# nelpy/ghost

Hardware: AMD Instinct MI355X
Metric: Msamples/s CWT (128ch x 1e6 samp x 100 scales); % HBM roofline; 1/2/4/8 GPU (higher is better)
Workload: dtype f32

## Files before the change

ghost_amd/csrc/api.cpp:

```cpp
#include <hip/hip_runtime.h>

#include <algorithm>
#include <cmath>
#include <cstdio>
#include <cstdlib>
#include <cstring>
#include <exception>
#include <map>
#include <new>
#include <string>
#include <vector>

#include "../../include/ghostcwt.h"
#include "../../include/ghostcwt_debug.h"
#include <memory>

#include "host_out.h"
#include "interp.h"
#include "kernels.h"
#include "morse_exact.h"
#include "options.h"
#include "planner.h"

using namespace gcwt;
// ... 18 lines not shown
  try {
    return body();
  } catch (const std::bad_alloc&) {
    return set_err(GCWT_ERR_NOMEM, "out of host memory");
  } catch (const std::exception& e) {
    return set_err(GCWT_ERR_INVALID, std::string("internal error: ") + e.what());
  } catch (...) {
    return set_err(GCWT_ERR_INVALID, "internal error");
  }
}

#define HIP_TRY(call)                                  \
  do {                                                 \
    hipError_t e_ = (call);                            \
    if (e_ != hipSuccess) return hip_err(e_, #call);   \
  } while (0)

struct EpochDev {
  SynthItemDev* items = nullptr;
  int n_items = 0;
  SynthLevelDev* levels = nullptr;
  Synth7Item* items7 = nullptr;
  Synth7Level* levels7 = nullptr;
  int n_items7 = 0;
  Synth7Item* items7w = nullptr;
  int n_items7w = 0;
  Synth7Item* items7n = nullptr;
  int n_items7n = 0;
  SynthiItem* items_i = nullptr;
  SynthiLevel* levels_i = nullptr;
  int n_items_i = 0;
  SynthpItem* items_p[2] = {nullptr, nullptr};
  SynthpLevel* levels_p = nullptr;
  int n_items_p[2] = {0, 0};
  PredLevel* pred_levels = nullptr;
};

constexpr int64_t kFullbandCacheBytes = (int64_t)16 << 30;

enum Stage { ST_MEAN = 0, ST_FWD, ST_DECIM, ST_BLOCK, ST_SYNTH, ST_DIRECT, ST_FULLBAND, ST_INTERP, ST_BLOCKCONV, ST_COUNT };

}

struct gcwt_plan {
  HostPlan hp;
  bool uploaded = false;
  int profiling = 0;
  int synth_cols = 32;
  int synth7_narrow_r = 2;
  bool fuse_blocks = true;
  int synth_kernel = 7;
  bool prune_inputs = true;
  bool fast_fft = true;
  int drop_stores = 0;
  bool clock_probe = false;
  bool use_synth16 = false;
  int device = -1;
  hipStream_t stream = nullptr;
  hipStream_t aux[2] = {nullptr, nullptr};
  bool level_streams = true;
  bool use_synthp = false;
  bool use_graphs = true;
  bool fullband4 = true;
  int fullband_group = 0;
  int64_t fullband_cache_cap = 0;
  bool hfull_cache_full = false;
  int synth7_order = 0;
  int synthp_help = -1;
  int synthp_lgnb = -1;
  int interp_lgnb = -1;
  int interp_grid = -1;
  bool last_fold = false;
  bool fold_mean = true;
  bool synth_streams = false;
  hipStream_t cur = nullptr;
  bool high_precision = true;
  double2* d_y = nullptr;
  int64_t y_stride = 0;
  double2* d_tw64 = nullptr;
  float2* d_x = nullptr;
  float2* d_xr = nullptr;
  float2* d_xb = nullptr;
  float2* d_bank = nullptr;
  float* d_gain = nullptr;
  float* d_gain_lv = nullptr;
  float2* d_half_tw = nullptr;
  float2* d_psi = nullptr;
  float2* d_psi_tail = nullptr;
  float2* d_psi_lit = nullptr;
  unsigned long long* d_probe = nullptr;
  double* d_amps = nullptr;
  float2* d_xs = nullptr;
  int64_t xs_stride = 0;
  float2* d_z = nullptr;
  int64_t z_half = 0;
  int z_sets = 1;
  float2* d_hfull = nullptr;
  std::map<std::pair<int, int>, float2*> hfull_cache;
  int64_t hfull_cache_bytes = 0;
  float2* d_tw4096 = nullptr;
  float2* d_tw256 = nullptr;
  float2* d_level_tw = nullptr;
  double* d_sums = nullptr;
  int32_t* d_scale_list = nullptr;
  int n_listed = 0;
  int32_t* d_scale_aux = nullptr;
// ... 196 lines not shown
  if (!free_bytes || !total_bytes) return set_err(GCWT_ERR_INVALID, "NULL argument");
  HIP_TRY(hipMemGetInfo(free_bytes, total_bytes));
  return GCWT_OK;
}
int gcwt_device_malloc(void** ptr, size_t bytes) { HIP_TRY(hipMalloc(ptr, bytes ? bytes : 1)); return GCWT_OK; }
int gcwt_device_free(void* ptr) { HIP_TRY(hipFree(ptr)); return GCWT_OK; }
int gcwt_memcpy_h2d(void* dst, const void* src, size_t bytes) {
  HIP_TRY(hipMemcpy(dst, src, bytes, hipMemcpyHostToDevice)); return GCWT_OK;
}
int gcwt_memcpy_d2h(void* dst, const void* src, size_t bytes) {
  HIP_TRY(hipMemcpy(dst, src, bytes, hipMemcpyDeviceToHost)); return GCWT_OK;
}
int gcwt_device_memset(void* dst, int value, size_t bytes) {
  HIP_TRY(hipMemset(dst, value, bytes)); return GCWT_OK;
}
int gcwt_device_synchronize(void) { HIP_TRY(hipDeviceSynchronize()); return GCWT_OK; }
int gcwt_host_alloc(void** ptr, size_t bytes) {
  if (!ptr) return set_err(GCWT_ERR_INVALID, "NULL argument");
  HIP_TRY(hipHostMalloc(ptr, bytes ? bytes : 1, hipHostMallocDefault));
  return GCWT_OK;
}
int gcwt_host_free(void* ptr) { HIP_TRY(hipHostFree(ptr)); return GCWT_OK; }
int gcwt_rows_to_host(const float* d_src, int64_t src_pitch, int64_t n_rows, int64_t row_elems, void* dst,
                      int64_t dst_pitch, int flags) {
  return guarded([&] {
    if (!d_src || !dst) return set_err(GCWT_ERR_INVALID, "NULL argument");
    if (n_rows < 0 || row_elems < 0 || src_pitch < row_elems || dst_pitch < row_elems)
      return set_err(GCWT_ERR_INVALID, "bad rectangle (rows, elements per row, pitches)");
    if (!(flags & GCWT_HOST_PINNED) && dst_pitch != row_elems)
      return set_err(GCWT_ERR_INVALID, "a destination that is not page-locked takes dense rows (dst_pitch = row_elems)");
    HIP_TRY(rows_to_host(d_src, src_pitch, n_rows, row_elems, dst, dst_pitch, (flags & GCWT_OUT_F64) != 0,
                         (flags & GCWT_HOST_PINNED) != 0));
    return (int)GCWT_OK;
  });
}

static int gcwt_plan_create_impl(gcwt_plan** out, const gcwt_params* params) {
  if (!out || !params) return set_err(GCWT_ERR_INVALID, "NULL argument");
  *out = nullptr;
  std::unique_ptr<gcwt_plan> owner(new (std::nothrow) gcwt_plan());
  gcwt_plan* p = owner.get();
  if (!p) return set_err(GCWT_ERR_NOMEM, "out of host memory");
  std::string err;
  int rc = build_host_plan(*params, &p->hp, &err);
  if (rc != GCWT_OK) return set_err(rc, err);
  p->hp.prm.freqs_hz = p->hp.freqs.data();
  p->hp.prm.epoch_bounds = p->hp.bounds.data();
  p->hp.prm.n_epochs = (int32_t)(p->hp.bounds.size() / 2);
  p->device = params->device;
  p->high_precision = p->hp.high_precision;
  p->use_synth16 = option_or("synth16", 0) == 1;
  p->synth_cols = option_or("synth_cols", 32) == 16 ? 16 : 32;
  p->synth7_narrow_r = (int)option_or("synth7_narrow_r", 2);
  p->fuse_blocks = option_or("fuse_blocks", 1) != 0;
  p->prune_inputs = option_or("prune_inputs", 1) != 0;
  p->fast_fft = option_or("slow_fft", 0) == 0;
  p->level_streams = option_or("level_streams", 1) != 0;
  if (option_is_set("interp_grid")) p->interp_grid = option_or("interp_grid", 0) != 0;
  p->synth_streams = option_or("synth_streams", 0) != 0;
  p->fold_mean = option_or("fold_mean", 1) != 0;
  p->interp_lgnb = (int)option_or("interp_lgnb", -1);
  p->use_synthp = kMeasureBuild && option_or("synthp", 0) != 0;
  p->synthp_lgnb = (int)option_or("synthp_lgnb", -1);
  p->synthp_help = (int)option_or("synthp_help", -1);
  p->use_graphs = option_or("graphs", 1) != 0;
  p->synth7_order = (int)option_or("synth7_order", 0);
  p->auto_threshold = 1e-9f * (float)option_or("auto_threshold_ppb", 1500);
  p->kappa_eps = 1e-9f * (float)option_or("auto_kappa_ppb", 160);
  p->oob_tol = 1e-12f * (float)option_or("auto_oob_ppt", 25000);
  p->fullband_group = (int)option_or("fullband_group", 0);
  p->fullband4 = option_or("fullband4", 1) != 0;
  p->synth_kernel = kMeasureBuild && option_or("synth_kernel", 7) == 8 ? 8 : 7;
  p->drop_stores = kMeasureBuild && option_is_set("synth_drop_stores") ? (int)std::max<long long>(1, option_or("synth_drop_stores", 1)) : 0;
  p->clock_probe = kMeasureBuild && option_is_set("clock_probe");
  for (const auto& s : p->hp.scales)
    if (s.method == GCWT_SCALE_DIRECT) p->max_direct_len = std::max(p->max_direct_len, s.length);
  *out = owner.release();
  return GCWT_OK;
}

void gcwt_plan_destroy(gcwt_plan* plan) {
  if (!plan) return;
  if (plan->uploaded || plan->stream) {
    if (plan->device >= 0) (void)hipSetDevice(plan->device);
    free_dev(plan);
  }
  delete plan;
}

int gcwt_plan_get_info(const gcwt_plan* plan, gcwt_plan_info* info) {
  if (!plan || !info) return set_err(GCWT_ERR_INVALID, "NULL argument");
  const HostPlan& hp = plan->hp;
  info->abi_version = GCWT_ABI_VERSION;
  info->n_levels = (int32_t)hp.levels.size();
  info->n_direct = hp.n_direct;
  info->n_spectral = (int32_t)hp.scales.size() - hp.n_direct - hp.n_fullband - hp.n_blockconv;
  info->n_fullband = hp.n_fullband;
  info->n_blockconv = hp.n_blockconv;
  info->reserved = 0;
  info->n_interp = 0;
  for (const auto& l : hp.levels)
    if (level_kernel(plan, l) == LK_INTERP) info->n_interp += (int32_t)l.scales.size();
  info->block = hp.block;
  int r = 1;
  for (const auto& l : hp.levels) r = std::max(r, l.decimation);
  info->max_decimation = r;
// ... 757 lines not shown
      ap.row_len = row_len;
      ap.xr = p->d_xr;
      ap.xr_cstride = hp.max_xr;
      ap.xb_scale = (float)(1.0 / ((double)hp.block * (double)Pt));
      ap.n_scales = S;
      ap.channels_fastest = p->interp_grid >= 0 ? p->interp_grid : (slots <= 32 ? 1 : 0);
      if (dev.n_items_p[k] > 65535) ap.channels_fastest = 0;
      ap.flags = 0;
      ap.seg = sout;
      p->cur = si;
#ifdef GCWT_MEASURE
      if (strided) return set_err(GCWT_ERR_UNSUPPORTED, "output stride with the pipelined interpolating kernel");
      RUN(ST_INTERP, launch_synthp(mode, ap, dev.n_items_p[k], slots, k == 1, si));
#else
      return set_err(GCWT_ERR_INVALID, "internal: a level planned for the measure build's pipelined kernel");
#endif
      p->cur = nullptr;
    }
    if (dev.n_items > 0) {
      SynthArgs a{};
      a.xb = p->d_xb;
      a.bank = p->d_bank;
      a.tw256 = p->d_tw256;
      a.level_tw = p->d_level_tw;
      a.items = dev.items;
      a.levels = dev.levels;
      a.out = dout;
      a.xb_cstride = hp.max_xb;
      a.row_len = row_len;
      a.n_scales = S;
      a.seg = sout;
      RUN(ST_SYNTH, launch_synth(mode, a, dev.n_items, slots, st));
    }
    for (int variant = 0; variant < 3; ++variant) {
      const int wide = variant == 2;
      const int cols7 = variant == 0 ? 16 : p->synth_cols;
      const int n7 = variant == 0 ? dev.n_items7n : wide ? dev.n_items7w : dev.n_items7;
      if (n7 == 0) continue;
      Synth7Args a7{};
      a7.xb = p->d_xb;
      a7.bank = p->d_bank;
      a7.tw256 = p->d_tw256;
      a7.level_tw = p->d_level_tw;
      a7.items = variant == 0 ? dev.items7n : wide ? dev.items7w : dev.items7;
      a7.levels = dev.levels7;
      a7.scale_list = p->d_scale_list;
      a7.gain = p->d_gain;
      a7.gain_lv = p->d_gain_lv;
      a7.level_half_tw = p->d_half_tw;
      a7.out = dout;
      a7.xb_cstride = hp.max_xb;
      a7.row_len = row_len;
      a7.n_scales = S;
      a7.drop_stores = p->drop_stores;
      a7.seg = sout;
      a7.clock_probe = p->d_probe;
      if (fused_blocks) {
        a7.xr = p->d_xr;
        a7.xr_cstride = hp.max_xr;
        a7.xb_scale = (float)(1.0 / ((double)hp.block * (double)Pt));
      }
      if (strided) {
        RUN(ST_SYNTH, launch_synth7s(mode, cols7, a7, n7, slots, st));
        continue;
      }
#ifdef GCWT_MEASURE
      if (p->synth_kernel == 8 && variant == 1)
        RUN(ST_SYNTH, launch_synth8(mode, p->synth_cols, a7, n7, slots, st));
      else
#endif
        RUN(ST_SYNTH, launch_synth7(mode, cols7, wide != 0, a7, n7, slots, st));
    }
    if (si != st) {
      hipEvent_t interp_done;
      int rc_ = get_event(p, &interp_done);
      if (rc_) return rc_;
      he = hipEventRecord(interp_done, si);
      if (he == hipSuccess) he = hipStreamWaitEvent(st, interp_done, 0);
      if (he != hipSuccess) return hip_err(he, "synthesis join");
    }
    if (p->detect && p->d_y) {
      hipEvent_t pred_done;
      int rc_ = get_event(p, &pred_done);
      if (rc_) return rc_;
      he = hipEventRecord(pred_done, p->det_stream);
      if (he == hipSuccess) he = hipStreamWaitEvent(st, pred_done, 0);
      if (he != hipSuccess) return hip_err(he, "detector join");
    }
    if (p->profiling && !hp.levels.empty()) p->last.synth_launches++;
    auto response = [&](int i, int scratch, const float2** h_out) -> int {
      const auto cached = p->hfull_cache.find({i, P1});
      if (cached != p->hfull_cache.end()) { *h_out = cached->second; return GCWT_OK; }
      float2* dst = p->d_hfull + (int64_t)scratch * hp.max_p;
      float2* keep = nullptr;
      const int64_t bytes = (int64_t)sizeof(float2) * P;
      if (!p->hfull_cache_full && p->hfull_cache_bytes + bytes <= p->fullband_cache_cap) {
        if (hipMalloc((void**)&keep, (size_t)bytes) == hipSuccess) dst = keep;
        else {
          (void)hipGetLastError();
          p->hfull_cache_full = true;
        }
      }
      {
        SpanGuard sg_(p, ST_FULLBAND);
        int rc_ = sg_.rc;
        if (!rc_) {
// ... 453 lines not shown

int gcwt_get_timings(const gcwt_plan* p, gcwt_timings* t) {
  if (!p || !t) return set_err(GCWT_ERR_INVALID, "NULL argument");
  if (!p->have_timings) return set_err(GCWT_ERR_INVALID, "no profiled execute yet");
  *t = p->last;
  return GCWT_OK;
}

int gcwt_plan_create(gcwt_plan** out, const gcwt_params* params) {
  return guarded([&] { return gcwt_plan_create_impl(out, params); });
}

int gcwt_plan_upload(gcwt_plan* p) {
  return guarded([&] { return gcwt_plan_upload_impl(p); });
}

int gcwt_execute(gcwt_plan* p, const void* x, void* out, int flags) {
  return guarded([&] { return gcwt_execute_impl(p, x, out, flags); });
}

int gcwt_execute_block(gcwt_plan* p, const void* x, void* out, int64_t start, int64_t length,
                       int flags) {
  return guarded([&] { return gcwt_execute_block_impl(p, x, out, start, length, flags); });
}


int gcwt_debug_measure_build(void) { return kMeasureBuild ? 1 : 0; }

int gcwt_debug_level_count(const gcwt_plan* p) { return p ? (int)p->hp.levels.size() : -1; }

int gcwt_debug_level_info(const gcwt_plan* p, int epoch, int level, int32_t* decimation,
                          int32_t* halo, int32_t* hop, int32_t* nblk, int64_t* m) {
  if (!p) return set_err(GCWT_ERR_INVALID, "NULL plan");
  if (epoch < 0 || epoch >= (int)p->hp.epochs.size() || level < 0 ||
      level >= (int)p->hp.levels.size())
    return set_err(GCWT_ERR_INVALID, "epoch/level out of range");
  const LevelPlan& lp = p->hp.levels[level];
  const EpochLevel& el = p->hp.epochs[epoch].lv[level];
  if (decimation) *decimation = lp.decimation;
  if (halo) *halo = lp.halo;
  if (hop) *hop = lp.hop;
  if (nblk) *nblk = el.nblk;
  if (m) *m = el.m;
  return GCWT_OK;
}

int gcwt_debug_level_band_shift(const gcwt_plan* p, int level, int32_t* shift) {
  if (!p || !shift) return set_err(GCWT_ERR_INVALID, "NULL argument");
  if (level < 0 || level >= (int)p->hp.levels.size()) return set_err(GCWT_ERR_INVALID, "level out of range");
  *shift = p->hp.levels[level].band_shift;
  return GCWT_OK;
}

int gcwt_debug_set_option(const char* name, int64_t value, int clear) {
  const int rc = option_set(name, (long long)value, clear != 0);
  if (rc == -1) return set_err(GCWT_ERR_INVALID, std::string("unknown option: ") + (name ? name : "(null)"));
  if (rc == -2) return set_err(GCWT_ERR_UNSUPPORTED, std::string("option ") + name + " exists in libghostcwt_measure.so only");
  return GCWT_OK;
}

int gcwt_debug_level_low_cut(const gcwt_plan* p, int level, double* theta_cut) {
  if (!p || !theta_cut) return set_err(GCWT_ERR_INVALID, "NULL argument");
  if (level < 0 || level >= (int)p->hp.levels.size()) return set_err(GCWT_ERR_INVALID, "level out of range");
  const LevelPlan& own = p->hp.levels[p->hp.levels[level].xr_owner];
  *theta_cut = p->hp.high_precision && own.band_shift == 0 ? own.taper_hi : 0.0;
  return GCWT_OK;
}

int gcwt_debug_scale_theta_lo(const gcwt_plan* p, double* theta_lo) {
  if (!p || !theta_lo) return set_err(GCWT_ERR_INVALID, "NULL argument");
  for (size_t i = 0; i < p->hp.scales.size(); ++i) theta_lo[i] = p->hp.scales[i].theta_lo;
  return GCWT_OK;
}

int gcwt_debug_mean_folded(const gcwt_plan* p) {
  if (!p) return set_err(GCWT_ERR_INVALID, "NULL plan");
  return p->last_fold ? 1 : 0;
}

int gcwt_debug_graph_state(const gcwt_plan* p) {
  if (!p) return set_err(GCWT_ERR_INVALID, "NULL plan");
  return p->graph_failed ? -1 : p->graph_exec ? 1 : 0;
}

int gcwt_debug_blockconv_groups(const gcwt_plan* p, int32_t* first, int32_t* count, int32_t* hop, int32_t* back,
                                int32_t* order, int max_groups, int max_order) {
  if (!p) return set_err(GCWT_ERR_INVALID, "NULL plan");
  const HostPlan& hp = p->hp;
  const int n = (int)hp.bc_groups.size();
  for (int g = 0; g < n && g < max_groups; ++g) {
    if (first) first[g] = hp.bc_groups[g].first;
    if (count) count[g] = hp.bc_groups[g].count;
    if (hop) hop[g] = hp.bc_groups[g].hop;
    if (back) back[g] = hp.bc_groups[g].back;
  }
  if (order) for (int k = 0; k < hp.n_blockconv && k < max_order; ++k) order[k] = hp.bc_order[k];
  return n;
}

int gcwt_debug_interp_level(const gcwt_plan* p, int level, int32_t* q, int32_t* factor, double* alpha,
                            double* err_bound, float* coef, int64_t max_floats) {
  if (!p) return set_err(GCWT_ERR_INVALID, "NULL plan");
  if (level < 0 || level >= (int)p->hp.levels.size()) return set_err(GCWT_ERR_INVALID, "level out of range");
  const LevelPlan& lp = p->hp.levels[level];
  const bool on = level_kernel(p, lp) == LK_INTERP;
  if (q) *q = on ? lp.interp_q : 0;
// ... 108 lines not shown
```

ghost_amd/csrc/kernels.h:

```cpp
#pragma once
#include <hip/hip_runtime.h>

#include <algorithm>
#include <cstdint>

#include "../../include/ghostcwt.h"

namespace gcwt {

constexpr int kRowLenDev = 4096;

#ifdef GCWT_MEASURE
constexpr bool kMeasureBuild = true;
#else
constexpr bool kMeasureBuild = false;
#endif

struct BankScale {
  double omega;
  double half_delay;
  int64_t length;
  int64_t amp_offset;
  int32_t bin_lo, n_bins;
  int32_t decimation;
// ... 59 lines not shown
  int32_t decimation, hop, halo, blk_base;
  int64_t xb_offset;
  int64_t tw_offset;
};

struct SynthArgs {
  const float2* xb;
  const float2* bank;
  const float2* tw256;
  const float2* level_tw;
  const SynthItemDev* items;
  const SynthLevelDev* levels;
  float* out;
  int64_t xb_cstride;
  int64_t row_len;
  int32_t n_scales;
  int32_t pad;
  SegOut seg;
};

struct Synth7Item {
  int32_t level, blk0, rtile, pad;
};

struct Synth7Level {
  int32_t decimation, log2r, hop, halo, nblk, n_scales, scale_offset, blk_base;
  int32_t n_plain;
  int32_t half_offset;
  int32_t band_shift;
  int32_t pad1;
  int64_t xb_offset;
  int64_t tw_offset;
  int64_t xr_offset;
  int64_t m_mask;
};

struct Synth7Args {
  const float2* xb;
  const float2* bank;
  const float2* tw256;
  const float2* level_tw;
  const Synth7Item* items;
  const Synth7Level* levels;
  const int32_t* scale_list;
  const float* gain;
  const float* gain_lv;
  const float2* level_half_tw;
  float* out;
  int64_t xb_cstride;
  int64_t row_len;
  const float2* xr;
  int64_t xr_cstride;
  float xb_scale;
  int32_t pad0;
  unsigned long long* clock_probe;
  int32_t n_scales;
  int32_t drop_stores;
  SegOut seg;
};

hipError_t launch_synth7(int mode, int ncol, bool wide_halo, const Synth7Args& a, int n_items, int n_channels,
                         hipStream_t st);
hipError_t launch_synth7s(int mode, int ncol, const Synth7Args& a, int n_items, int n_channels, hipStream_t st);

struct SynthiItem {
  int32_t level, blk0;
  int32_t pass0, n_pass;
  int32_t wt_lo, wt_hi;
};
struct SynthiLevel {
  int32_t decimation, q, log2q, factor;
  int32_t hop, halo, nblk, n_scales, scale_offset, blk_base;
  int32_t log2nb, taps;
  int64_t tw_offset;
  int64_t xr_offset;
  int64_t m_mask;
  int64_t coef_offset;
};
struct SynthiArgs {
  const float2* tw256;
  const float2* level_tw;
  const SynthiItem* items;
  const SynthiLevel* levels;
  const int32_t* scale_list;
  const int32_t* scale_aux;
  const float* gain;
  const float* coef;
  float* out;
  int64_t row_len;
  const float2* xr;
  int64_t xr_cstride;
  float xb_scale;
  int32_t n_scales;
  int32_t channels_fastest;
  SegOut seg;
};
hipError_t launch_synthi(int mode, const SynthiArgs& a, int n_items, int n_channels, hipStream_t st);
hipError_t launch_synthis(int mode, const SynthiArgs& a, int n_items, int n_channels, hipStream_t st);
constexpr int kSynthpThreads = 512;
constexpr int kSynthpProducers = 2;
constexpr int kSynthpSlots = 4;
constexpr int kSynthpMaxFactor = 256;
struct SynthpItem {
  int32_t level, blk0;
  int32_t round0, n_rounds;
};
struct SynthpLevel {
// ... 180 lines not shown
```

ghost_amd/csrc/options.cpp:

```cpp
#include "options.h"

#include <cctype>
#include <cstdlib>
#include <cstring>
#include <map>
#include <mutex>
#include <string>

#include "kernels.h"

namespace gcwt {
namespace {

const char* const kSelect[] = {"synth16", "synth_cols", "fuse_blocks", "slow_fft", "level_streams", "interp_grid",
                               "synth_streams", "interp_lgnb", "merge_levels", "split_levels", "interp",
                               "batch_bytes", "stage_floats", "fullband_group", "blockconv",
                               "direct_max_len", "graphs", "plan_threads", "fullband_cache_mb", "auto_threshold_ppb", "auto_kappa_ppb", "auto_oob_ppt", "synth7_order", "host_widen", "host_threads", "fullband4", "cu_count", "synth7_narrow_r", "fold_mean"};
const char* const kMeasureOnly[] = {"halo_margin", "interp_q", "interp_taps", "interp_min_r", "prune_inputs", "clock_phases",
                                    "synth_kernel", "synth_drop_stores", "clock_probe", "synthi_pad_kb",
                                    "synthp", "synthp_lgnb", "synthp_help"};
const char* const kEnvBudgets[] = {"batch_bytes", "stage_floats"};

std::mutex g_mu;
std::map<std::string, long long>& table() {
  static std::map<std::string, long long> t;
  return t;
}

template <size_t N>
bool in_list(const char* name, const char* const (&list)[N]) {
  for (const char* s : list)
    if (!strcmp(s, name)) return true;
  return false;
}

bool from_env(const char* name, long long* v) {
  std::string var = "GHOSTCWT_";
  for (const char* c = name; *c; ++c) var.push_back((char)toupper((unsigned char)*c));
  const char* e = getenv(var.c_str());
  if (!e) return false;
  *v = *e ? atoll(e) : 1;
  return true;
}

bool lookup(const char* name, long long* v) {
  {
    std::lock_guard<std::mutex> lock(g_mu);
    auto it = table().find(name);
    if (it != table().end()) { *v = it->second; return true; }
  }
  if (kMeasureBuild || in_list(name, kEnvBudgets)) return from_env(name, v);
  return false;
}

}

long long option_or(const char* name, long long dflt) {
  long long v;
  return lookup(name, &v) ? v : dflt;
}

bool option_is_set(const char* name) {
  long long v;
  return lookup(name, &v);
}

int option_set(const char* name, long long value, bool clear) {
  if (!name) return -1;
  const bool measure_only = in_list(name, kMeasureOnly);
  if (!measure_only && !in_list(name, kSelect)) return -1;
// ... 9 lines not shown
```

ghost_amd/csrc/planner.cpp:

```cpp
#include "planner.h"
#include "interp.h"
#include "morse_exact.h"
#include "options.h"

#include <algorithm>
#include <climits>
#include <cstdlib>
#include <cmath>
#include <map>
#include <atomic>
#include <mutex>
#include <new>
#include <thread>

namespace gcwt {

static int exact_method(const HostPlan& hp, int64_t length) {
  if (length <= hp.direct_max_len) return GCWT_SCALE_DIRECT;
  if (length <= hp.blockconv_max_len) return GCWT_SCALE_BLOCKCONV;
  return GCWT_SCALE_FULLBAND;
}
static bool uses_segment_fft(int method) { return method == GCWT_SCALE_SPECTRAL || method == GCWT_SCALE_FULLBAND; }

static void plan_blockconv(HostPlan* hp, bool rebalance) {
// ... 693 lines not shown
    if (sp.method != GCWT_SCALE_SPECTRAL) continue;
    const int r = sp.decimation;
    if (r > r_cap) return fail(GCWT_ERR_UNSUPPORTED, "internal: decimation beyond the shortest FFT");
    int halo = std::max((int)std::ceil(sp.support / (double)r) + halo_margin(), 16);
    if (r == 2) halo += halo & 1;
    const std::pair<int, int> key(r, sp.theta_neg > 0.0 && halo > 48 ? 2 : (split && halo > 16 ? 1 : 0));
    auto it = level_of.find(key);
    if (it == level_of.end()) {
      LevelPlan lp;
      lp.decimation = r;
      const int idx = (int)hp->levels.size();
      if (!owner_of_r.count(r)) owner_of_r[r] = idx;
      lp.xr_owner = owner_of_r[r];
      level_of[key] = idx;
      hp->levels.push_back(lp);
      it = level_of.find(key);
    }
    sp.level = it->second;
    LevelPlan& lp = hp->levels[sp.level];
    lp.scales.push_back(i);
    lp.halo = std::max(lp.halo, halo);
  }
  {
    std::map<int, int> shift_of_r;
    for (const LevelPlan& lp : hp->levels) {
      const double delta = 2.0 * M_PI / ((double)B * lp.decimation);
      int& shift = shift_of_r[lp.decimation];
      for (int i : lp.scales)
        if (hp->scales[i].theta_neg > 0.0)
          shift = std::max(shift, (int)std::ceil(hp->scales[i].theta_neg / delta));
    }
    for (LevelPlan& lp : hp->levels) {
      const double delta = 2.0 * M_PI / ((double)B * lp.decimation);
      const int g = std::max(1, lp.decimation / 16);
      const int shift = (shift_of_r[lp.decimation] + g - 1) / g * g;
      lp.band_shift = shift;
      for (int i : lp.scales)
        if (hp->scales[i].theta_hi > (double)(B - shift) * delta * (1.0 + 1e-12))
          return fail(GCWT_ERR_UNSUPPORTED, "internal: a scale's band does not fit its level's shifted band");
      if (shift > 0 && lp.scales.size() > 256)
        return fail(GCWT_ERR_UNSUPPORTED, "more than 256 heavy-tailed scales in one decimation level");
    }
  }
  if (hp->high_precision) {
    std::vector<double> lo(hp->levels.size(), 1e30);
    for (const LevelPlan& lp : hp->levels) {
      double& o = lo[(size_t)lp.xr_owner];
      if (lp.band_shift > 0) o = 0.0;
      for (int i : lp.scales) o = std::min(o, hp->scales[i].theta_lo);
    }
    for (size_t l = 0; l < hp->levels.size(); ++l)
      hp->levels[l].taper_hi = hp->levels[l].xr_owner == (int)l && lo[l] < 1e29 ? lo[l] : 0.0;
  }
  for (LevelPlan& lp : hp->levels) {
    lp.hop = B - 2 * lp.halo;
    if (lp.hop < 32)
      return fail(GCWT_ERR_UNSUPPORTED,
                  "internal: a spectral scale does not fit its 256-sample decimated block");
    lp.fast = lp.halo <= 48 && lp.scales.size() <= 256;
    if (!lp.fast) hp->halo_static = false;
    lp.twiddle_offset = hp->level_twiddle_total;
    hp->level_twiddle_total += (int64_t)kSynthCols * lp.decimation;
  }
  {
    if (option_or("interp", 1) != 0) {
      const size_t nl = hp->levels.size();
      std::vector<std::vector<float>> coef(nl);
      const unsigned n_thr = (unsigned)std::min<size_t>(nl, std::min<unsigned>((unsigned)std::max<long long>(1, option_or("plan_threads", 8)), std::max(1u, std::thread::hardware_concurrency())));
      if (n_thr <= 1) {
        for (size_t l = 0; l < nl; ++l) plan_interp_level(hp, &hp->levels[l], &coef[l]);
      } else {
        std::atomic<size_t> next{0};
        std::atomic<bool> failed{false};
        auto work = [&]() {
          try {
            for (size_t l = next++; l < nl; l = next++) plan_interp_level(hp, &hp->levels[l], &coef[l]);
          } catch (...) {
            failed = true;
          }
        };
        std::vector<std::thread> pool;
        try {
          for (unsigned k = 1; k < n_thr; ++k) pool.emplace_back(work);
        } catch (...) {
        }
        work();
        for (std::thread& t : pool) t.join();
        if (failed) throw std::bad_alloc();
      }
      for (size_t l = 0; l < nl; ++l) {
        if (hp->levels[l].interp_q <= 0 || coef[l].empty()) continue;
        hp->levels[l].coef_offset = (int64_t)hp->interp_coef.size();
        hp->interp_coef.insert(hp->interp_coef.end(), coef[l].begin(), coef[l].end());
      }
    }
  }

  for (const EpochPlan& ep : hp->epochs) {
    if (ep.long_a == 1) continue;
    if (!hp->high_precision)
      return fail(GCWT_ERR_UNSUPPORTED, "FFT lengths above 2^22 (kernels of millions of taps) need precision = high");
    if (hp->n_fullband > 0)
      return fail(GCWT_ERR_UNSUPPORTED, "FFT lengths above 2^22 cannot serve full-band scales (heavy-tailed wavelet at very low frequencies)");
    for (const LevelPlan& lp : hp->levels) {
      const int64_t m = ep.p / lp.decimation;
      if (lp.band_shift > 0 || lp.decimation < 2 * ep.long_a ||
          (lp.decimation / ep.long_a > kMaxTwoPassDecimation && m > 8192))
// ... 90 lines not shown
```

ghost_amd/csrc/planner.h:

```cpp
#pragma once
#include <cstdint>
#include <string>
#include <vector>

#include "../../include/ghostcwt.h"

namespace gcwt {

constexpr int kRowLen = 4096;
constexpr int kMaxP1 = 1024;
constexpr int kMaxFftLog2 = 24;
constexpr int kMaxDecimation = 16384;
constexpr int kMaxBatch = 16;
constexpr int kMaxTwoPassDecimation = 256;
constexpr int kSynthCols = 16;
constexpr int kSynthWide = 32;
constexpr int kDirectMaxLen = 256;
constexpr int kDirectDefaultLen = 48;
constexpr int kBlockConvRamp = 256;
constexpr int kBlockConvExactMaxLen = 1024;
constexpr int kBlockConvMaxLen = 2560;

struct ScalePlan {
  double freq_hz = 0, omega = 0;
  int64_t length = 0;
  int method = GCWT_SCALE_SPECTRAL;
  int decimation = 1;
  int level = -1;
  double half_delay = 0;
  int direct_index = -1;
  int64_t direct_offset = 0;
  int fullband_index = -1;
  int blockconv_index = -1;
  int32_t bin_lo = 0, n_bins = 0;
  int64_t amp_offset = 0;
  double theta_hi = 0;
  double theta_neg = 0;
  double theta_lo = 0;
  double support = 0;
  bool band_ok = false;
  int demod_bin = 0;
};

struct LevelPlan {
  int decimation = 1;
  int halo = 0;
  int hop = 0;
  std::vector<int> scales;
  bool fast = true;
  int xr_owner = -1;
  int64_t twiddle_offset = 0;
  int band_shift = 0;
  double taper_hi = 0;
  int interp_q = 0;
  int interp_taps = 8;
  int interp_factor = 0;
  int64_t coef_offset = 0;
  double interp_alpha = 0;
  double interp_err = 0;
};

struct EpochLevel {
  int64_t m = 0;
  int blk_lo = 0;
  int nblk = 0;
  int64_t xr_offset = 0;
  int64_t xb_offset = 0;
};

struct SynthItem {
  int32_t level, scale, blk0, nblk;
};

struct EpochPlan {
// ... 66 lines not shown
```

ghost_amd/csrc/synth.hip:

```cpp
#include <hip/hip_runtime.h>

#include "kernels.h"
#include "synth_math.h"

#ifndef GCWT_STORE_AUX
#define GCWT_STORE_AUX 2
#endif

namespace gcwt {

__device__ __forceinline__ v2f phase_carrier(int shift, int r, int R) {
  float sn, cs;
  sincospif(-2.0f * (float)(shift * r) / (256.0f * (float)R), &sn, &cs);
  return (v2f){cs, sn};
}

template <int STRIDE>
__device__ __forceinline__ void twiddle_to_planes(v2f* exw, const v2f (&v)[16], const v2f* tw, int stride = STRIDE) {
  const int st = STRIDE ? STRIDE : stride;
#pragma unroll
  for (int jj = 0; jj < 8; ++jj) {
    const v4f w2 = *reinterpret_cast<const v4f*>(tw + 2 * jj);
    exw[(2 * jj) * st] = jj == 0 ? v[0] : cmulv(v[dft16_pos(2 * jj)], (v2f){w2.x, w2.y});
    exw[(2 * jj + 1) * st] = cmulv(v[dft16_pos(2 * jj + 1)], (v2f){w2.z, w2.w});
// ... 130 lines not shown
    }
  } else {
    const int blk = min(it.blk0 + blk_l, lv.nblk - 1);
    const float2* xb = a.xb + (int64_t)c * a.xb_cstride + lv.xb_offset + (int64_t)blk * 256 + t;
    v2f wcur = (v2f){b0.x, b0.y};
    if (sh) {
      const float2 cb = a.tw256[(-(int64_t)sh * ((int64_t)(lv.blk_base + blk) * hop - halo)) & 255];
      wcur = cmulv(cmulv(wcur, phase_carrier(sh, r, R)), (v2f){cb.x, cb.y});
    }
    const v2f wstep = (v2f){st.x, st.y};
#pragma unroll
    for (int j = 0; j < 16; ++j) {
      const float2 q = xb[16 * j];
      pw[j] = cmulv((v2f){q.x, q.y}, wcur);
      wcur = cmulv(wcur, wstep);
    }
    if (tid < lv.n_scales) sc_lds[tid] = sc_v;
    if (tid < 256) { twl[(tid & 15) * kTwPitch + (tid >> 4)] = (v2f){tw_v.x, tw_v.y}; half_lds[tid] = (v2f){half_v.x, half_v.y}; }
    park_gains();
    if (lv.n_scales > kChunk) load_gains(kChunk);
  }
  const int sstride = wide ? NCOL : R;
  v2f* const exw = ex + ((t - sh) & 15) * kPlane + (wide ? colw : (blk_l << (4 + lg)) + r);
  const int blk_l2 = wide ? 0 : (tid >> (4 + lg));
  const int rem = wide ? tid : (tid & ((16 << lg) - 1));
  const int m2 = wide ? (tid >> kLgN) : (rem >> lg);
  const int r2 = wide ? it.rtile * NCOL + (tid & (NCOL - 1)) : (rem & (R - 1));
  const v2f* const exr = ex + tid;
  const int off0 = (blk_l2 * hop + m2 - halo) * R + r2;
  const int m1step = 16 * R;
  const bool deep = halo > 32;
  const bool keep1 = !deep && m2 >= halo - 16, keep14 = !deep && m2 < 32 - halo;
  const bool keep2 = !deep || m2 >= halo - 32, keep13 = !deep || m2 < 48 - halo;
  unsigned keep_rows = 0;
  if (WIDE) {
#pragma unroll
    for (int m1 = 0; m1 < 16; ++m1) keep_rows |= (16 * m1 + m2 >= halo && 16 * m1 + m2 < 256 - halo) ? 1u << m1 : 0u;
  }

  constexpr int kElem = MODE == GCWT_OUT_COMPLEX_C64 ? 2 : 1;
  const int64_t n_b = (int64_t)(lv.blk_base + it.blk0) * hop * R;
  const int64_t w_lo = a.seg.w_lo[seg];
  const int64_t w_len = a.seg.w_hi[seg] - w_lo;
  const unsigned ext_bytes = w_len > 0 && !(kMeasureBuild && (a.drop_stores & 1)) ? (unsigned)(w_len * (4 * kElem)) : 0u;
  float* const out0 = a.out + ((int64_t)ch * a.n_scales * a.row_len + a.seg.seg_col[seg] + w_lo) * kElem;
  const unsigned voff0 = (unsigned)(((int)(n_b - w_lo) + off0) * (4 * kElem));
  const unsigned vstep = (unsigned)(m1step * (4 * kElem));
  const bool pair_rows = !wide && lg == 1;
  const bool upper = (tid & 32) != 0;
  const bool keep_p0 = upper ? keep2 : keep1, keep_p6 = upper ? keep14 : keep13;
  const unsigned voff_pair = voff0 - (upper ? (unsigned)((2 * hop - 32) * 4) : 0u);
  const unsigned pair_step = (unsigned)(2 * hop * 4);
  const float* const st_rd = stage + t * 20;
  __syncthreads();
  if (kMeasureBuild && a.clock_probe) probe_ph[3] = __builtin_amdgcn_s_memrealtime();

  for (int b = 0; b < lv.n_scales; ++b) {
    if (b > 0 && (b & (kChunk - 1)) == 0) {
      __syncthreads();
      park_gains();
      if (b + kChunk < lv.n_scales) load_gains(b + kChunk);
      __syncthreads();
    }
    if (b == lv.n_plain) {
#pragma unroll
      for (int j = 0; j < 16; ++j) pw[j] = cmulv(pw[j], half_lds[t + 16 * j]);
    }
    const float4* const hs = reinterpret_cast<const float4*>(st_rd + (b & (kChunk - 1)) * kGainRow);
    const int entry = __builtin_amdgcn_readfirstlane(sc_lds[b]);
    v2f v[16];
    switch ((unsigned)entry >> 24) {
#define GCWT_WINDOW(hi) case 16 - (hi): gain_first_layer<hi>(v, pw, hs); break;
      GCWT_WINDOW(15) GCWT_WINDOW(14) GCWT_WINDOW(13) GCWT_WINDOW(12) GCWT_WINDOW(11) GCWT_WINDOW(10) GCWT_WINDOW(9)
#undef GCWT_WINDOW
      default: gain_first_layer<16>(v, pw, hs); break;
    }
    idft16v_tail(v);
    switch (sstride) {
      case 2: twiddle_to_planes<2>(exw, v, twl + t * kTwPitch); break;
      case 4: twiddle_to_planes<4>(exw, v, twl + t * kTwPitch); break;
      case 8: twiddle_to_planes<8>(exw, v, twl + t * kTwPitch); break;
      case 16: twiddle_to_planes<16>(exw, v, twl + t * kTwPitch); break;
      case 32: twiddle_to_planes<32>(exw, v, twl + t * kTwPitch); break;
      default: twiddle_to_planes<0>(exw, v, twl + t * kTwPitch, sstride); break;
    }
    if (!(kMeasureBuild && (a.drop_stores & 2))) __syncthreads();
#pragma unroll
    for (int k1 = 0; k1 < 16; ++k1) v[k1] = exr[k1 * kPlane];
    if (!(kMeasureBuild && (a.drop_stores & 2))) __syncthreads();
    idft16v(v);

    const int srow = entry & kScaleIndexMask;
    const uint64_t dst_bits = reinterpret_cast<uint64_t>(out0 + (int64_t)srow * a.row_len * kElem);
    const uint32_t dst_lo = __builtin_amdgcn_readfirstlane((uint32_t)dst_bits);
    const uint32_t dst_hi = __builtin_amdgcn_readfirstlane((uint32_t)(dst_bits >> 32));
    float* const dst = reinterpret_cast<float*>(((uint64_t)dst_hi << 32) | dst_lo);
    const __amdgpu_buffer_rsrc_t rsrc = __builtin_amdgcn_make_buffer_rsrc(
        dst, 0, __builtin_amdgcn_readfirstlane(ext_bytes), 0x00020000);
    if (MODE != GCWT_OUT_COMPLEX_C64 && !WIDE && pair_rows) {
#pragma unroll
      for (int m1 = 1; m1 < 15; m1 += 2) {
        const v2f z0 = v[dft16_pos(m1)], z1 = v[dft16_pos(m1 + 1)];
        const float p0 = __builtin_fmaf(z0.y, z0.y, z0.x * z0.x), p1 = __builtin_fmaf(z1.y, z1.y, z1.x * z1.x);
        const float a0 = MODE == GCWT_OUT_AMPLITUDE_F32 ? __builtin_amdgcn_sqrtf(p0) : p0;
        const float a1 = MODE == GCWT_OUT_AMPLITUDE_F32 ? __builtin_amdgcn_sqrtf(p1) : p1;
        const auto sw = __builtin_amdgcn_permlane32_swap(__builtin_bit_cast(unsigned, a0),
                                                         __builtin_bit_cast(unsigned, a1), false, false);
        const bool keep = m1 == 1 ? keep_p0 : m1 == 13 ? keep_p6 : true;
        const unsigned vo = voff_pair + (unsigned)m1 * vstep;
        if (keep) {
          __builtin_amdgcn_raw_buffer_store_b32(sw[0], rsrc, vo, 0, GCWT_STORE_AUX);
          __builtin_amdgcn_raw_buffer_store_b32(sw[1], rsrc, vo + pair_step, 0, GCWT_STORE_AUX);
        }
      }
      continue;
    }
#pragma unroll
    for (int m1 = 1; m1 < 15; ++m1) {
      const v2f z = v[dft16_pos(m1)];
      const bool keep = WIDE ? (keep_rows >> m1) & 1u
                             : m1 == 1 ? keep1 : m1 == 2 ? keep2 : m1 == 13 ? keep13 : m1 == 14 ? keep14 : true;
      const unsigned vo = voff0 + (unsigned)m1 * vstep;
      if (MODE == GCWT_OUT_COMPLEX_C64) {
        typedef unsigned v2u __attribute__((ext_vector_type(2)));
        if (keep) __builtin_amdgcn_raw_buffer_store_b64(__builtin_bit_cast(v2u, z), rsrc, vo, 0, GCWT_STORE_AUX);
      } else {
        const float p2 = __builtin_fmaf(z.y, z.y, z.x * z.x);
        const float val = MODE == GCWT_OUT_AMPLITUDE_F32 ? __builtin_amdgcn_sqrtf(p2) : p2;
        if (keep) __builtin_amdgcn_raw_buffer_store_b32(__builtin_bit_cast(unsigned, val), rsrc, vo, 0, GCWT_STORE_AUX);
      }
    }
  }
  if (kMeasureBuild && a.clock_probe && tid == 0) {
    atomicAdd(a.clock_probe, (unsigned long long)(__builtin_amdgcn_s_memtime() - probe_c0));
    atomicAdd(a.clock_probe + 1, (unsigned long long)(__builtin_amdgcn_s_memrealtime() - probe_t0));
    for (int i = 0; i < 4; ++i) atomicAdd(a.clock_probe + 2 + i, (unsigned long long)(probe_ph[i] - probe_t0));
    atomicAdd(a.clock_probe + 6, 1ull);
  }
}

template <int NCOL, bool WIDE>
static hipError_t launch_synth7_n(int mode, const Synth7Args& a, int n_items, int n_channels,
                                  hipStream_t st) {
  constexpr int lds = 16 * (16 * NCOL + 1) * 8 + 16 * 18 * 8 + 8 * 320 * 4 + 256 * 4 + 256 * 8;
  static bool attr_done[64] = {};
  int dev_ = 0;
  (void)hipGetDevice(&dev_);
  bool& attr_set = attr_done[dev_ & 63];
  if (!attr_set) {
    hipError_t e = hipFuncSetAttribute((const void*)k_synth7<GCWT_OUT_AMPLITUDE_F32, NCOL, WIDE>,
                                       hipFuncAttributeMaxDynamicSharedMemorySize, lds);
    if (e != hipSuccess) return e;
    e = hipFuncSetAttribute((const void*)k_synth7<GCWT_OUT_POWER_F32, NCOL, WIDE>,
                            hipFuncAttributeMaxDynamicSharedMemorySize, lds);
    if (e != hipSuccess) return e;
    e = hipFuncSetAttribute((const void*)k_synth7<GCWT_OUT_COMPLEX_C64, NCOL, WIDE>,
                            hipFuncAttributeMaxDynamicSharedMemorySize, lds);
    if (e != hipSuccess) return e;
    attr_set = true;
  }
  dim3 grid(n_items, n_channels), block(16 * NCOL);
  if (mode == GCWT_OUT_AMPLITUDE_F32)
    hipLaunchKernelGGL((k_synth7<GCWT_OUT_AMPLITUDE_F32, NCOL, WIDE>), grid, block, lds, st, a);
  else if (mode == GCWT_OUT_POWER_F32)
    hipLaunchKernelGGL((k_synth7<GCWT_OUT_POWER_F32, NCOL, WIDE>), grid, block, lds, st, a);
  else
    hipLaunchKernelGGL((k_synth7<GCWT_OUT_COMPLEX_C64, NCOL, WIDE>), grid, block, lds, st, a);
  return hipGetLastError();
}

hipError_t launch_synth7(int mode, int ncol, bool wide_halo, const Synth7Args& a, int n_items, int n_channels,
                         hipStream_t st) {
  if (n_items == 0) return hipSuccess;
  if (wide_halo)
    return ncol == 16 ? launch_synth7_n<16, true>(mode, a, n_items, n_channels, st)
                      : launch_synth7_n<32, true>(mode, a, n_items, n_channels, st);
  return ncol == 16 ? launch_synth7_n<16, false>(mode, a, n_items, n_channels, st)
                    : launch_synth7_n<32, false>(mode, a, n_items, n_channels, st);
}

}
```

include/ghostcwt_debug.h:

```cpp
#ifndef GHOSTCWT_DEBUG_H
#define GHOSTCWT_DEBUG_H
#include "ghostcwt.h"
#ifdef __cplusplus
extern "C" {
#endif

enum {
  GCWT_DEBUG_SPECTRUM = 0,
  GCWT_DEBUG_DECIMATED = 1,
  GCWT_DEBUG_BLOCK_SPECTRA = 2
};

int gcwt_debug_set_option(const char* name, int64_t value, int clear);
int gcwt_debug_level_count(const gcwt_plan* plan);
int gcwt_debug_level_info(const gcwt_plan* plan, int epoch, int level, int32_t* decimation,
                          int32_t* halo, int32_t* hop, int32_t* nblk, int64_t* m);
int gcwt_debug_level_band_shift(const gcwt_plan* plan, int level, int32_t* shift);
int gcwt_debug_level_low_cut(const gcwt_plan* plan, int level, double* theta_cut);
int gcwt_debug_scale_theta_lo(const gcwt_plan* plan, double* theta_lo);
int gcwt_debug_graph_state(const gcwt_plan* plan);
int gcwt_debug_mean_folded(const gcwt_plan* plan);
int gcwt_debug_precision_terms(gcwt_plan* plan, float* rounding, float* left_out, float* level_energy,
                               float* band_energy);
int gcwt_debug_blockconv_groups(const gcwt_plan* plan, int32_t* first, int32_t* count, int32_t* hop,
                                int32_t* back, int32_t* order, int max_groups, int max_order);
int gcwt_debug_batch_of(const gcwt_plan* plan, int segment, int32_t* first, int32_t* count);
int gcwt_debug_fetch(gcwt_plan* plan, int what, int channel, int epoch, int level, float* dst,
                     int64_t max_complex);
int gcwt_debug_exact_gain(const gcwt_plan* plan, int scale, const int64_t* a, int64_t b, int64_t n,
                          double* gain);
int gcwt_debug_interp_level(const gcwt_plan* plan, int level, int32_t* q, int32_t* factor,
                            double* alpha, double* err_bound, float* coef, int64_t max_floats);
int gcwt_debug_scale_demod(const gcwt_plan* plan, int32_t* demod);
int gcwt_debug_scale_theta_neg(const gcwt_plan* plan, double* theta_neg);
int gcwt_debug_measure_build(void);
int gcwt_debug_clock(gcwt_plan* plan, double* ghz, double* workgroup_seconds);
enum { GCWT_BW_FILL = 0, GCWT_BW_COPY = 1, GCWT_BW_SYNTH_STORES = 2,
       GCWT_BW_SYNTHI_STORES = 3  };
int gcwt_debug_bandwidth(int pattern, size_t bytes, double* gb_per_s);

int gcwt_debug_check_output(const void* out_device, int64_t row_pitch_floats, int64_t n_valid_floats,
                            int32_t rows_per_channel, int32_t n_channels, int32_t distinct,
                            int64_t* n_nonfinite, int64_t* n_mismatched);

#ifdef __cplusplus
}
#endif
#endif
```

Baseline: 9389.

## Use wave-local barriers in synth7 exchange and align halos to cache lines

```diff
diff --git a/ghost_amd/csrc/api.cpp b/ghost_amd/csrc/api.cpp
--- a/ghost_amd/csrc/api.cpp
+++ b/ghost_amd/csrc/api.cpp
@@ -94,6 +94,7 @@
   int synth_kernel = 7;
   bool prune_inputs = true;
   bool fast_fft = true;
+  int synth7_wave_sync = 1;
   int drop_stores = 0;
   bool clock_probe = false;
   bool use_synth16 = false;
@@ -396,6 +397,7 @@
   p->use_synth16 = option_or("synth16", 0) == 1;
   p->synth_cols = option_or("synth_cols", 32) == 16 ? 16 : 32;
   p->synth7_narrow_r = (int)option_or("synth7_narrow_r", 2);
+  p->synth7_wave_sync = option_or("synth7_wave_sync", 1) != 0;
   p->fuse_blocks = option_or("fuse_blocks", 1) != 0;
   p->prune_inputs = option_or("prune_inputs", 1) != 0;
   p->fast_fft = option_or("slow_fft", 0) == 0;
@@ -1259,6 +1261,7 @@
       a7.xb_cstride = hp.max_xb;
       a7.row_len = row_len;
       a7.n_scales = S;
+      a7.wave_sync = p->synth7_wave_sync;
       a7.drop_stores = p->drop_stores;
       a7.seg = sout;
       a7.clock_probe = p->d_probe;
@@ -1818,6 +1821,8 @@
   return GCWT_OK;
 }
 
+int gcwt_debug_line_aligned_halo(int decimation, int halo) { return line_aligned_halo(decimation, halo); }
+
 int gcwt_debug_set_option(const char* name, int64_t value, int clear) {
   const int rc = option_set(name, (long long)value, clear != 0);
   if (rc == -1) return set_err(GCWT_ERR_INVALID, std::string("unknown option: ") + (name ? name : "(null)"));
diff --git a/ghost_amd/csrc/kernels.h b/ghost_amd/csrc/kernels.h
--- a/ghost_amd/csrc/kernels.h
+++ b/ghost_amd/csrc/kernels.h
@@ -135,7 +135,7 @@
   const float2* xr;
   int64_t xr_cstride;
   float xb_scale;
-  int32_t pad0;
+  int32_t wave_sync;
   unsigned long long* clock_probe;
   int32_t n_scales;
   int32_t drop_stores;
diff --git a/ghost_amd/csrc/options.cpp b/ghost_amd/csrc/options.cpp
--- a/ghost_amd/csrc/options.cpp
+++ b/ghost_amd/csrc/options.cpp
@@ -15,7 +15,8 @@
 const char* const kSelect[] = {"synth16", "synth_cols", "fuse_blocks", "slow_fft", "level_streams", "interp_grid",
                                "synth_streams", "interp_lgnb", "merge_levels", "split_levels", "interp",
                                "batch_bytes", "stage_floats", "fullband_group", "blockconv",
-                               "direct_max_len", "graphs", "plan_threads", "fullband_cache_mb", "auto_threshold_ppb", "auto_kappa_ppb", "auto_oob_ppt", "synth7_order", "host_widen", "host_threads", "fullband4", "cu_count", "synth7_narrow_r", "fold_mean"};
+                               "direct_max_len", "graphs", "plan_threads", "fullband_cache_mb", "auto_threshold_ppb", "auto_kappa_ppb", "auto_oob_ppt", "synth7_order", "host_widen", "host_threads", "fullband4", "cu_count", "synth7_narrow_r", "fold_mean",
+                               "synth7_wave_sync", "align_runs"};
 const char* const kMeasureOnly[] = {"halo_margin", "interp_q", "interp_taps", "interp_min_r", "prune_inputs", "clock_phases",
                                     "synth_kernel", "synth_drop_stores", "clock_probe", "synthi_pad_kb",
                                     "synthp", "synthp_lgnb", "synthp_help"};
diff --git a/ghost_amd/csrc/planner.cpp b/ghost_amd/csrc/planner.cpp
--- a/ghost_amd/csrc/planner.cpp
+++ b/ghost_amd/csrc/planner.cpp
@@ -769,7 +769,9 @@
     for (size_t l = 0; l < hp->levels.size(); ++l)
       hp->levels[l].taper_hi = hp->levels[l].xr_owner == (int)l && lo[l] < 1e29 ? lo[l] : 0.0;
   }
+  const bool align_runs = option_or("align_runs", 1) != 0;
   for (LevelPlan& lp : hp->levels) {
+    if (align_runs) lp.halo = line_aligned_halo(lp.decimation, lp.halo, B);
     lp.hop = B - 2 * lp.halo;
     if (lp.hop < 32)
       return fail(GCWT_ERR_UNSUPPORTED,
diff --git a/ghost_amd/csrc/planner.h b/ghost_amd/csrc/planner.h
--- a/ghost_amd/csrc/planner.h
+++ b/ghost_amd/csrc/planner.h
@@ -20,6 +20,13 @@
 constexpr int kBlockConvRamp = 256;
 constexpr int kBlockConvExactMaxLen = 1024;
 constexpr int kBlockConvMaxLen = 2560;
+
+inline int line_aligned_halo(int r, int halo, int block = 256) {
+  if ((r != 2 && r != 4) || halo > 32) return halo;
+  int h = halo;
+  while (h <= 32 && ((block - 2 * h) * r * 4) % 128 != 0) ++h;
+  return h <= 32 ? h : halo;
+}
 
 struct ScalePlan {
   double freq_hz = 0, omega = 0;
diff --git a/ghost_amd/csrc/synth.hip b/ghost_amd/csrc/synth.hip
--- a/ghost_amd/csrc/synth.hip
+++ b/ghost_amd/csrc/synth.hip
@@ -206,9 +206,23 @@
   const unsigned voff_pair = voff0 - (upper ? (unsigned)((2 * hop - 32) * 4) : 0u);
   const unsigned pair_step = (unsigned)(2 * hop * 4);
   const float* const st_rd = stage + t * 20;
+  const bool wave_local = a.wave_sync && !wide && lg <= 2;
   __syncthreads();
   if (kMeasureBuild && a.clock_probe) probe_ph[3] = __builtin_amdgcn_s_memrealtime();
 
+#pragma unroll
+  for (int kind = 0; kind < 2; ++kind) {
+  if ((kind != 0) != wave_local) continue;
+  auto exchange_sync = [&]() {
+    if (kMeasureBuild && (a.drop_stores & 2)) return;
+    if (kind != 0) {
+      __builtin_amdgcn_fence(__ATOMIC_RELEASE, "wavefront");
+      __builtin_amdgcn_wave_barrier();
+      __builtin_amdgcn_fence(__ATOMIC_ACQUIRE, "wavefront");
+    } else {
+      __syncthreads();
+    }
+  };
   for (int b = 0; b < lv.n_scales; ++b) {
     if (b > 0 && (b & (kChunk - 1)) == 0) {
       __syncthreads();
@@ -238,10 +252,10 @@
       case 32: twiddle_to_planes<32>(exw, v, twl + t * kTwPitch); break;
       default: twiddle_to_planes<0>(exw, v, twl + t * kTwPitch, sstride); break;
     }
-    if (!(kMeasureBuild && (a.drop_stores & 2))) __syncthreads();
+    exchange_sync();
 #pragma unroll
     for (int k1 = 0; k1 < 16; ++k1) v[k1] = exr[k1 * kPlane];
-    if (!(kMeasureBuild && (a.drop_stores & 2))) __syncthreads();
+    exchange_sync();
     idft16v(v);
 
     const int srow = entry & kScaleIndexMask;
@@ -284,6 +298,7 @@
         if (keep) __builtin_amdgcn_raw_buffer_store_b32(__builtin_bit_cast(unsigned, val), rsrc, vo, 0, GCWT_STORE_AUX);
       }
     }
+  }
   }
   if (kMeasureBuild && a.clock_probe && tid == 0) {
     atomicAdd(a.clock_probe, (unsigned long long)(__builtin_amdgcn_s_memtime() - probe_c0));
diff --git a/include/ghostcwt_debug.h b/include/ghostcwt_debug.h
--- a/include/ghostcwt_debug.h
+++ b/include/ghostcwt_debug.h
@@ -12,6 +12,7 @@
 };
 
 int gcwt_debug_set_option(const char* name, int64_t value, int clear);
+int gcwt_debug_line_aligned_halo(int decimation, int halo);
 int gcwt_debug_level_count(const gcwt_plan* plan);
 int gcwt_debug_level_info(const gcwt_plan* plan, int epoch, int level, int32_t* decimation,
                           int32_t* halo, int32_t* hop, int32_t* nblk, int64_t* m);
```

After: 9402, median of 6. About the same (+0.1%).
